# ZJU-FAST-Lab/uneven_planner

Hardware: AMD Instinct MI355X
Metric: MINCO traj-opts/sec (batch) (higher is better)
Workload: dtype f64

## Files before the change

### uneven_planner_amd/csrc/map_build.hip

```cpp
#include <hip/hip_runtime.h>
#include <hipcub/hipcub.hpp>
#include <sys/stat.h>

#include <algorithm>
#include <cmath>
#include <cstdint>
#include <chrono>
#include <cstdio>
#include <cstring>
#include <mutex>
#include <string>
#include <thread>
#include <vector>

#include "../../include/uneven_hip.h"
#include "uph_internal.hpp"
#include "terrain_dev.hpp"
#include "rccl_dyn.hpp"

using namespace uph;

struct uph_map {
    int device = 0;
    uph_map_params mp;
// ... 565 lines not shown
    g.xy_inv = 1.0 / g.xy_res; g.yaw_inv = 1.0 / g.yaw_res;
    for (int i = 0; i < 3; i++) { g.minb[i] = -size[i] / 2.0; g.maxb[i] = size[i] / 2.0; g.origin[i] = g.minb[i]; }
    finishGrid(g);
    g.nx = (int)std::ceil(size[0] / g.xy_res); g.ny = (int)std::ceil(size[1] / g.xy_res); g.nyaw = (int)std::ceil(size[2] / g.yaw_res);
    g.gravity = mp->gravity;
    if (tx1 < 0) tx1 = g.nx;
    if (tx0 < 0 || tx1 > g.nx || tx0 >= tx1) { delete m; setError("uph_map_create_tile: bad x-range"); return UPH_ERR_INVALID; }
    g.x_off = tx0; g.nx_hold = tx1 - tx0;
    m->ncell = (size_t)g.nx_hold * g.ny * g.nyaw;
    if (m->ncell >= ((size_t)1 << 31)) { setError("uph_map_create: more than 2^31 cells held by one device (the lookups index cells with 32 bits): use tiles"); delete m; return UPH_ERR_LIMIT; }
    g.cells = nullptr; g.cells32 = nullptr;
    int r = UPH_OK;
    auto alloc = [&](void** p, size_t bytes) { if (r == UPH_OK && hipMalloc(p, bytes) != hipSuccess) { setError("uph_map_create: hipMalloc of the grid failed"); r = UPH_ERR_HIP; } };
    if (f32) {
        alloc((void**)&m->d_cells32, m->ncell * 4 * sizeof(float));
        if (r == UPH_OK && hipMemset(m->d_cells32, 0, m->ncell * 4 * sizeof(float)) != hipSuccess) r = UPH_ERR_HIP;
        g.cells32 = m->d_cells32;
    } else {
        alloc((void**)&m->d_cells, m->ncell * 4 * sizeof(double));
        alloc((void**)&m->d_c, m->ncell * sizeof(double));
        if (r == UPH_OK && hipMemset(m->d_cells, 0, m->ncell * 4 * sizeof(double)) != hipSuccess) r = UPH_ERR_HIP;
        g.cells = m->d_cells;
    }
    alloc((void**)&m->d_occ, m->ncell);
    alloc((void**)&m->d_occ2, (size_t)g.nx_hold * g.ny);
    if (r == UPH_OK) r = commitMap(m);
    if (r != UPH_OK) { uph_map_destroy(m); return r; }
    *out = m;
    return UPH_OK;
}

int uph_map_create(const uph_map_params* mp, int device, uph_map** out) { return createMap(mp, device, out, false); }
int uph_map_create_f32(const uph_map_params* mp, int device, uph_map** out) { return createMap(mp, device, out, true); }
int uph_map_create_tile(const uph_map_params* mp, int device, int32_t x0, int32_t x1, int32_t f32, uph_map** out) { return createMap(mp, device, out, f32 != 0, x0, x1); }
int uph_map_tile(const uph_map* m, int32_t* x0, int32_t* x1) {
    if (!m || !x0 || !x1) return UPH_ERR_INVALID;
    *x0 = m->g.x_off; *x1 = m->g.x_off + m->g.nx_hold;
    return UPH_OK;
}
int uph_map_storage_bytes(const uph_map* m) { return !m ? UPH_ERR_INVALID : (m->d_cells32 ? 4 : 8); }

void uph_map_destroy(uph_map* m) {
    if (!m) return;
    hipSetDevice(m->device);
    hipFree(m->d_cells); hipFree(m->d_cells32); hipFree(m->d_c); hipFree(m->d_occ); hipFree(m->d_occ2);
    for (int k = 0; k < 4; k++) hipFree(m->scratch[k]);
// ... 688 lines not shown
```

### uneven_planner_amd/csrc/solver_program.hpp

```cpp
#pragma once
#include "terrain_dev.hpp"
#include "trajectory_dev.hpp"
#include "uph_common.hpp"

namespace uph {

#ifndef UPH_GRID_FROM_MEM
#define UPH_GRID_FROM_MEM 1
#endif
#ifndef UPH_PHASE_MASK
#define UPH_PHASE_MASK 15
#endif
#ifndef UPH_SCALING_WB
#define UPH_SCALING_WB 8
#endif
#ifndef UPH_SC_XB
#define UPH_SC_XB 9
#endif
#ifndef UPH_SC_YB
#define UPH_SC_YB 14
#endif
#ifndef UPH_SC_WLO
#define UPH_SC_WLO 2
#endif
#ifndef UPH_SC_WHI
#define UPH_SC_WHI 3
#endif

template <class WG, class SR = double>
struct Solver {
    WG& wg;
    const GridDev& grid;
    const OptParams& P;
    const BatchDev& bd;
    const TrajDesc& td;
    int Nxy, Nyaw, n, S, K, mem, CH, CHP, recd;
    int CHS;
// ... 300 lines not shown
    UPH_HD void putRec(int slot, int i, int j, const R gp_[2], const R gv_[2], const R ga_[2], R gyaw, R gdyaw, const KinT<R>& k) {
        rec[0 * CHP + slot] = gp_[0]; rec[1 * CHP + slot] = gp_[1];
        rec[2 * CHP + slot] = gv_[0]; rec[3 * CHP + slot] = gv_[1];
        rec[4 * CHP + slot] = ga_[0]; rec[5 * CHP + slot] = ga_[1];
        R u1 = k.u;
        if (UPH_DIET) pinv(u1);
        const R u2 = u1 * u1, u3 = u2 * u1, u4 = u2 * u2, u5 = u4 * u1;
        rec[6 * CHP + slot] = gyaw;
        rec[7 * CHP + slot] = (u1 * gyaw + gdyaw);
        rec[8 * CHP + slot] = (u2 * gyaw + 2.0 * u1 * gdyaw);
        rec[9 * CHP + slot] = (u3 * gyaw + 3.0 * u2 * gdyaw);
        rec[10 * CHP + slot] = (u4 * gyaw + 4.0 * u3 * gdyaw);
        rec[11 * CHP + slot] = (u5 * gyaw + 5.0 * u4 * gdyaw);
        rtag[slot] = k.yaw_idx;
        if (i == 0) {
            double* w = wtab + 6 * j;
            R s1 = k.s1;
            if (UPH_DIET) pinv(s1);
            const R s2 = s1 * s1, s3 = s2 * s1, s4 = s2 * s2, s5 = s4 * s1;
            w[0] = 1.0; w[1] = s1; w[2] = s2; w[3] = s3; w[4] = s4; w[5] = s5;
        }
    }

    template <int RES, class R = double>
    UPH_HD void sampleEval(int s, int slot, double* acc) {
        constexpr bool RES_ONLY = RES == 1;
        UPH_MARK("sampleEval");
        const int i = divSmall(s, K + 1, inv_k1), j = s - i * (K + 1);
        R dl[7], sc7[7];
#if !defined(UPH_LATE_DUALS) || !UPH_LATE_DUALS
#pragma unroll
        for (int q = 0; q < 7; q++) { dl[q] = R(RES_ONLY ? 0.0 : dual[q * S + s]); sc7[q] = R(scl[q * S + s]); }
#endif
        KinT<R> k;
        kin<false, R>(i, j, k);
        UPH_MARK("sampleEval.penalties");
#if defined(UPH_LATE_DUALS) && UPH_LATE_DUALS
        {
            int s_ = s;
            asm volatile("" : "+v"(s_));
#pragma unroll
            for (int q = 0; q < 7; q++) { dl[q] = R(RES_ONLY ? 0.0 : dual[q * S + s_]); sc7[q] = R(scl[q * S + s_]); }
        }
#endif
        const R icvx = k.tv[0], icvy = k.tv[2], cos_xi = k.tv[4], icxi = k.tv[5], sigma = k.tv[6];
        const R vx = k.vx, wz = k.wz, ax = k.ax, ay = k.ay, curv = k.curv_snorm;
        const R nh0 = k.syaw, nh1 = -k.cyaw;
#if defined(__HIP_DEVICE_COMPILE__) && UPH_GRID_FROM_MEM
        typedef const __attribute__((address_space(4))) unsigned long long* pw_t;
        pw_t PT = (pw_t)(const void*)bd.params_mem;
        asm volatile("" : "+s"(PT));
        constexpr int PWORD = (int)(sizeof(OptParams) / 8);
        unsigned long long pw[PWORD];
#pragma unroll
        for (int q = 0; q < PWORD; q++) pw[q] = PT[q];
        OptParams Pm;
        __builtin_memcpy(&Pm, pw, sizeof(OptParams));
#else
        const OptParams& Pm = P;
#endif
        const R h = (k.vel[0] * nh0 + k.vel[1] * nh1) * sc7[0];
        const R g1 = (vx * vx - Pm.max_vel2) * sc7[1];
        const R g2 = (ax * ax - Pm.max_acc_lon2) * sc7[2];
        const R g3 = (ay * ay - Pm.max_acc_lat2) * sc7[3];
        const R sc4 = Pm.use_scaling ? sc7[4] : R(cur_scale);
// ... 362 lines not shown
        double sm[3] = {0.0, 0.0, 0.0};
        for (int s0 = 0; s0 < S; s0 += CHS) {
            const int cnt = S - s0 < CHS ? S - s0 : CHS;
            double part[3];
            wg.template sum<3>(cnt, part, [&](int t, double* acc) { sampleObjective(s0 + t, t, acc); });
            sm[0] += part[0]; sm[1] += part[1]; sm[2] += part[2];
            scatterChunk(s0, cnt);
        }
        double chx, chy;
        adjoint(chx, chy);
        const double gTau_fx = (P.rho_T + (js[1] + sm[1] + chx) / Nxy + (js[2] + sm[2] + chy) / Nyaw) * dTau;
        const double mq = wg.maxv((Nxy - 1) * 2 + (Nyaw - 1), [&](int t) {
            return t < (Nxy - 1) * 2 ? fabs(gamxy[3 * 2 + t]) : fabs(gamyaw[3 + (t - (Nxy - 1) * 2)]);
        });
        scale_fx = wg.bcast(1.0 / dmax(1.0, dmax(mq, fabs(gTau_fx))));
        wg.pfor(2, [&](int u) { fillTimes(u); });
        wg.pfor(S, [&](int s) { scalingSample(s, dTau); });
    }

    UPH_HD void scalingSample(int s, double dTau) {
        const int i = divSmall(s, K + 1, inv_k1), j = s - i * (K + 1);
        Kin k;
        kin(i, j, k);
#if !defined(UPH_SCALING_GROUPS) || UPH_SCALING_GROUPS == 2
        scalingGroup<0, 4>(s, i, j, k, dTau);
        scalingGroup<4, 3>(s, i, j, k, dTau);
#elif UPH_SCALING_GROUPS == 3
        scalingGroup<0, 3>(s, i, j, k, dTau);
        scalingGroup<3, 2>(s, i, j, k, dTau);
        scalingGroup<5, 2>(s, i, j, k, dTau);
#else
        scalingGroup<0, 7>(s, i, j, k, dTau);
#endif
    }
    template <int Q0, int NQS>
    UPH_HD void scalingGroup(int s, int i, int j, const Kin& k, double dTau) {
        const int nbx = Nxy + 5, nby = Nyaw + 5;
        const double Tx = Txy, Ty = Tyaw, itx = 1.0 / Txy, ity = 1.0 / Tyaw;
        const double gravity = grid.gravity;
        const double alpha = 1.0 / K * j;
        const double icvx = k.tv[0], icvy = k.tv[2], icxi = k.tv[5];
        const int m = k.yaw_idx;
        double dpL[NQS][2], dvL[NQS][2], daL[NQS][2], dpR[NQS][2], dvR[NQS][2], daR[NQS][2];
        double ypL[NQS], yvL[NQS], yaL[NQS], ypR[NQS], yvR[NQS], yaR[NQS];
        double sumx[NQS], sumy[NQS], mx[NQS];
#pragma unroll
        for (int qi = 0; qi < NQS; qi++) {
// ... 312 lines not shown
        wg.pfor(S, [&](int s) {
            dual[s] += r * res[s];
            for (int q = 1; q < 7; q++) dual[q * S + s] = dmax(dual[q * S + s] + r * res[q * S + s], 0.0);
        });
        rho = wg.bcast(dmin((1 + P.gamma) * rho, P.beta));
    }
    UPH_HD bool judgeConvergence() {
        const double r = rho;
        const double rh = wg.maxv(S, [&](int s) { return fabs(res[s]); });
        const double rg = wg.maxv(6 * S, [&](int t) { return fabs(dmax(res[S + t], -dual[S + t] / r)); });
        return dmax(rh, rg) < P.epsilon_con;
    }

    UPH_HD void storeTrajectory(TrajState& st) {
        double* oc = bd.cxy + td.off_cxy;
        double* oy = bd.cyaw + td.off_cyaw;
        wg.pfor(12 * Nxy + 6 * Nyaw, [&](int t) { if (t < 12 * Nxy) oc[t] = cxy[t]; else oy[t - 12 * Nxy] = cyaw[t - 12 * Nxy]; });
        wg.pfor(1, [&](int) {
            st.T_xy = Txy; st.T_yaw = Tyaw; st.jerk_cost = last_jerk; st.scale_fx = scale_fx; st.rho = rho;
            st.evals = evals; st.hist_reads = hist_reads;
#ifdef UPH_TL_PROF
            for (int q = 0; q < 6; q++) cyc[8 + q] = wg.tl[q];
#endif
            for (int q = 0; q < 16; q++) st.cyc[q] = cyc[q];
        });
#ifdef UPH_BAR_PROF
        wg.sync();
        wg.dumpBar(&st.cyc[8]);
#endif
    }

    UPH_HD void prepare(TrajState& st) {
        const double* gx0 = bd.x0 + td.off_x;
        double* gx = bd.x + td.off_x;
        rho = wg.bcast(st.rho);
        scale_fx = 1.0;
        wg.pfor(S > n ? S : n, [&](int t) {
            if (t < n) { x[t] = gx0[t]; gx[t] = gx0[t]; }
            if (t < S) for (int q = 0; q < 7; q++) { dual[q * S + t] = 0.0; res[q * S + t] = 0.0; scl[q * S + t] = 1.0; }
        });
        const long long tstart = wg.clock();
        if (P.use_scaling) initScaling(x);
        cyc[5] += wg.clock() - tstart;
        wg.pfor(1, [&](int) { st.scale_fx = scale_fx; st.cyc[5] = cyc[5]; });
    }

    UPH_HD void optimize(TrajState& st, int cap = 0) {
// ... 211 lines not shown
```

### uneven_planner_amd/csrc/terrain_dev.hpp

```cpp
#pragma once
#include "uph_common.hpp"


namespace uph {

template <class R>
struct CornersT {
    R dx, dy, dyaw;
    uint32_t a[2][2];
    int w0, w1;
    bool inmap;
};
typedef CornersT<double> Corners;

template <class R>
UPH_HD bool isInMap(const GridDev& g, R x, R y, R yaw) {
    if (x < g.lo[0] || y < g.lo[1] || yaw < g.lo[2]) return false;
    if (x > g.hi[0] || y > g.hi[1] || yaw > g.hi[2]) return false;
    return true;
}

UPH_HD int clampIdx(int v, int hi) { return v < 0 ? 0 : (v > hi ? hi : v); }

template <class R>
// ... 39 lines not shown
    typedef const __attribute__((address_space(1))) double* wordp;
#else
    struct dbl2_t { double x, y; };
    struct flt4_t { float x, y, z, w; };
    typedef const dbl2_t* cellp;
    typedef const flt4_t* cellp32;
    typedef const double* wordp;
#endif
    if (F32) {
        const flt4_t v = ((cellp32)g.cells32)[idx];
        f[3] = toReal<R>(v.x); f[0] = toReal<R>(v.y); f[1] = toReal<R>(v.z); f[2] = toReal<R>(v.w);
    } else if (WITH_Z) {
        const cellp p = (cellp)(g.cells + 4 * (size_t)idx);
        const dbl2_t lo = p[0], hi = p[1];
        f[3] = lo.x; f[0] = lo.y; f[1] = hi.x; f[2] = hi.y;
    } else {
        const double* p = g.cells + 4 * (size_t)idx;
        const double sg = ((wordp)p)[1];
        const dbl2_t hi = ((cellp)p)[1];
        f[3] = R(0.0); f[0] = sg; f[1] = hi.x; f[2] = hi.y;
    }
}

template <bool GRAD, bool WITH_Z, class R, class CELLS>
UPH_HD void interpCellsWith(const GridDev& g, R dx, R dy, R dw, CELLS cells, R val[4], R grd[3][3]) {
    constexpr int NF = WITH_Z ? 4 : 3;
    R v0[NF], v1[NF], gy0[3], gy1[3], gx[3];
#pragma unroll
    for (int w = 0; w < 2; w++) {
        R f[2][2][4];
        cells(w, f);
#pragma unroll
        for (int k = 0; k < NF; k++) {
            const R vy0 = f[0][0][k] * (1 - dx) + f[1][0][k] * dx;
            const R vy1 = f[0][1][k] * (1 - dx) + f[1][1][k] * dx;
            const R vv = vy0 * (1 - dy) + vy1 * dy;
            if (w == 0) v0[k] = vv; else v1[k] = vv;
            if (GRAD && k < 3) {
                const R gxa = f[1][0][k] - f[0][0][k], gxb = f[1][1][k] - f[0][1][k];
                if (w == 0) { gy0[k] = vy1 - vy0; gx[k] = (1 - dw) * (1 - dy) * gxa; gx[k] += (1 - dw) * dy * gxb; }
                else { gy1[k] = vy1 - vy0; gx[k] += dw * (1 - dy) * gxa; gx[k] += dw * dy * gxb; }
            }
        }
    }
#pragma unroll
    for (int k = 0; k < NF; k++) {
        val[k] = v0[k] * (1 - dw) + v1[k] * dw;
        if (GRAD && k < 3) {
            grd[k][2] = (v1[k] - v0[k]) * g.yaw_inv;
            grd[k][1] = (gy0[k] * (1 - dw) + gy1[k] * dw) * g.xy_inv;
            grd[k][0] = gx[k] * g.xy_inv;
        }
    }
}
template <bool F32, bool GRAD, bool WITH_Z, class R>
UPH_HD void interpCells(const GridDev& g, const CornersT<R>& c, R val[4], R grd[3][3]) {
    interpCellsWith<GRAD, WITH_Z, R>(g, c.dx, c.dy, c.dyaw, [&](int w, R f[2][2][4]) {
        const int wi = w == 0 ? c.w0 : c.w1;
#pragma unroll
        for (int a = 0; a < 2; a++)
#pragma unroll
            for (int b = 0; b < 2; b++) loadCell<F32, R, WITH_Z>(g, c.a[a][b] + (uint32_t)wi, f[a][b]);
    }, val, grd);
}

template <class R>
UPH_HD void terrainBase(const GridDev& g, R x, R y, R yaw, R& sg, R& zx, R& zy, R gs[3], R gzx[3], R gzy[3]) {
    CornersT<R> c;
    locate<R>(g, x, y, yaw, c);
    sg = R(0.0); zx = R(0.0); zy = R(0.0);
#pragma unroll
    for (int k = 0; k < 3; k++) { gs[k] = R(0.0); gzx[k] = R(0.0); gzy[k] = R(0.0); }
    if (!c.inmap) return;
    R val[4], grd[3][3];
    if (g.cells32) interpCells<true, true, false, R>(g, c, val, grd);
    else interpCells<false, true, false, R>(g, c, val, grd);
    sg = val[0]; zx = val[1]; zy = val[2];
#pragma unroll
    for (int k = 0; k < 3; k++) { gs[k] = grd[0][k]; gzx[k] = grd[1][k]; gzy[k] = grd[2][k]; }
}

UPH_HD void terrainValues(const GridDev& g, const Corners& c, double val[4]) {
    val[0] = val[1] = val[2] = val[3] = 0.0;
    if (!c.inmap) return;
    double grd[3][3];
    if (g.cells32) interpCells<true, false, true, double>(g, c, val, grd);
    else interpCells<false, false, true, double>(g, c, val, grd);
}

UPH_HD void terrainAllWithGrad(const GridDev& g, double x, double y, double yaw, double cyaw, double syaw,
                               double values[7], double grads[7][3]) {
    double sg, zx, zy, gs[3], gzx[3], gzy[3];
    terrainBase(g, x, y, yaw, sg, zx, zy, gs, gzx, gzy);
    double cc = sqrt(1.0 - zx * zx - zy * zy);
    double gc[3];
#pragma unroll
    for (int k = 0; k < 3; k++) gc[k] = -(gzx[k] * zx + gzy[k] * zy) / cc;
    double inv_c = 1.0 / cc;
// ... 68 lines not shown
```

### uneven_planner_amd/csrc/unevenhip.hip

```cpp
#include <hip/hip_runtime.h>

#include <type_traits>

#include <algorithm>
#include <cmath>
#include <cstdio>
#include <cstdlib>
#include <cstring>
#include <map>
#include <numeric>
#include <string>
#include <thread>
#include <vector>

#include "../../include/uneven_hip.h"
#include "minco_op_host.hpp"
#include "resample_walk.hpp"
#include "solver_program.hpp"
#include "uph_internal.hpp"

using namespace uph;

#ifndef UPH_THOMAS_KPL
#define UPH_THOMAS_KPL 4
#endif
#ifndef UPH_WPS128
#define UPH_WPS128 2
#endif
#ifndef UPH_TWOLOOP_PF
#define UPH_TWOLOOP_PF 5
#endif

template <int CTRL>
__device__ __forceinline__ double dppMov(double v) {
    const int lo = __builtin_amdgcn_mov_dpp(__double2loint(v), CTRL, 0xf, 0xf, false);
    const int hi = __builtin_amdgcn_mov_dpp(__double2hiint(v), CTRL, 0xf, 0xf, false);
    return __hiloint2double(hi, lo);
}
__device__ __forceinline__ double readLane(double v, int l) {
    return __hiloint2double(__builtin_amdgcn_readlane(__double2hiint(v), l), __builtin_amdgcn_readlane(__double2loint(v), l));
}
__device__ __forceinline__ int uni(int v) { return __builtin_amdgcn_readfirstlane(v); }
__device__ __forceinline__ double uni(double v) {
    return __hiloint2double(__builtin_amdgcn_readfirstlane(__double2hiint(v)), __builtin_amdgcn_readfirstlane(__double2loint(v)));
}
typedef const __attribute__((address_space(1))) double* gcptr;
__device__ __forceinline__ gcptr uniG(const double* p) {
    const unsigned long long a = (unsigned long long)p;
    const unsigned lo = __builtin_amdgcn_readfirstlane((unsigned)a), hi = __builtin_amdgcn_readfirstlane((unsigned)(a >> 32));
    return (gcptr)(((unsigned long long)hi << 32) | lo);
// ... 462 lines not shown
            else if (nq == 7) twoLoopT<7, 2>(d, g, dg_out, al_lds, n, hist, m, end, bound, scale);
            else twoLoopT<8, 2>(d, g, dg_out, al_lds, n, hist, m, end, bound, scale);
            __builtin_amdgcn_s_setprio(0);
        }
        bar(1);
    }
    template <class F>
    __device__ __forceinline__ double maxv(int n, F f) {
        double a = 0.0;
        for (int i = ftid(); i < n; i += NT) { const double v = f(i); a = v > a ? v : a; }
        a = waveMax(a);
        double* r = red + par * (NW * MAXM);
        par ^= 1;
        if (lane == 0) r[wave * MAXM] = a;
        bar(0);
        double t = r[0];
#pragma unroll
        for (int w = 1; w < NW; w++) t = r[w * MAXM] > t ? r[w * MAXM] : t;
        return uni(t);
    }
};

template <int NT, int WPS, int MODE, bool F32S = false>
__global__ __launch_bounds__(NT, WPS) void uph_solver_kernel(GridDev grid, OptParams P, BatchDev bd, int repeat) {
    extern __shared__ double lds[];
    const int w = blockIdx.x;
    if (w >= bd.B) return;
    const int b = bd.order ? bd.order[w] : w;
    DevWG<NT> wg(lds);
    typedef typename std::conditional<F32S, f32r, double>::type SR;
    Solver<DevWG<NT>, SR> sol(wg, grid, P, bd, b, lds + DevWG<NT>::SCRATCH);
    TrajState& st = bd.state[b];
    if (MODE == 0) sol.evalOnly(st, repeat);
    else if (MODE == 1) sol.prepare(st);
    else if (MODE == 2) sol.optimize(st, repeat);
    else if (MODE == 7) sol.resumeHook(st, repeat >> 1, repeat & 1);
    else if (MODE == 8) { if (repeat & 1) sol.template penaltyOnly<true>(st, repeat >> 1); else sol.template penaltyOnly<false>(st, repeat >> 1); }
    else if (MODE == 3) sol.report(st);
    else if (MODE == 5) sol.microbench(st, repeat);
    else sol.scalingOnly(st);
}

__global__ void uph_fill_kernel(double* __restrict__ p, size_t n, double v) {
    for (size_t i = (size_t)blockIdx.x * blockDim.x + threadIdx.x; i < n; i += (size_t)gridDim.x * blockDim.x) p[i] = v;
}

__global__ void uph_terrain_kernel(GridDev grid, const double* __restrict__ pos, int n, double* __restrict__ values, double* __restrict__ grads) {
    const int i = blockIdx.x * blockDim.x + threadIdx.x;
    if (i >= n) return;
    const double yaw = pos[3 * i + 2];
    double v[7], g[7][3];
    terrainAllWithGrad(grid, pos[3 * i], pos[3 * i + 1], yaw, cos(yaw), sin(yaw), v, g);
    for (int k = 0; k < 7; k++) {
        values[7 * i + k] = v[k];
        for (int q = 0; q < 3; q++) grads[21 * i + 3 * k + q] = g[k][q];
    }
}

struct RolloutTraj {
    int64_t row0;
    int cnt, rows;
    double total;
    double shift[2];
// ... 219 lines not shown
    for (int k = 0; k < r.nxy; k++) {
        const double* w = states + (size_t)(r.row_xy + k) * TRAJ_STATE_COLS;
        for (int d = 0; d < 2; d++) {
            oxy[2 * k + d] = w[d];
            h.lo[d] = w[d] < h.lo[d] ? w[d] : h.lo[d];
            h.hi[d] = h.hi[d] < w[d] ? w[d] : h.hi[d];
        }
    }
    double* oyw = st_yaw + (size_t)r.q * PLAN_SY;
    double prev = h.yaw_init;
    for (int k = 0; k <= r.nyw; k++) {
        const double cur = k < r.nyw ? states[(size_t)(r.row_yaw + k) * TRAJ_STATE_COLS + 9] : h.yaw_end;
        if (k < r.nyw) oyw[k] = cur;
        const double dy = fabs(cur - prev);
        h.turn += dy; h.kink = h.kink < dy ? dy : h.kink; prev = cur;
    }
    heads[r.q] = h;
}

#ifdef UPH_ONE_KERNEL
#ifndef UPH_OK_F32
#define UPH_OK_F32 false
#endif
template __global__ void uph_solver_kernel<UPH_OK_NT, UPH_OK_WPS, UPH_OK_MODE, UPH_OK_F32>(GridDev, OptParams, BatchDev, int);
#else
namespace uph {
thread_local std::string g_last_error;
void setError(const std::string& s) { g_last_error = s; }
}

struct DevBuf {
    void* p = nullptr;
    size_t cap = 0;
    int ensure(size_t bytes) {
        if (bytes <= cap) return 0;
        if (p) hipFree(p);
        p = nullptr; cap = 0;
        size_t want = bytes + bytes / 4 + 256;
        if (hipMalloc(&p, want) != hipSuccess) { setError("hipMalloc failed"); return -1; }
        cap = want;
        return 0;
    }
    void release() { if (p) hipFree(p); p = nullptr; cap = 0; }
    template <class T> T* as() { return (T*)p; }
};

struct HostBuf {
// ... 40 lines not shown
    size_t lds_big = 0;
    int n_main = 0;
    std::vector<int> rejected;
    int n_rejected = 0;
    bool all_rejected = false;
    std::vector<TrajFrame> frames;
    std::vector<GridDev> grid_host_framed;
    GridDev frames_grid;
    GridDev framed_from;
    bool framed_valid = false;
    std::vector<int> origin;
    bool sample_f32 = false;
    int xcd_group = 0;
    hipStream_t stream2 = nullptr;
    hipEvent_t evp0 = nullptr, evp1 = nullptr;
    bool pending = false;
    hipEvent_t ev2 = nullptr;
    std::vector<size_t> fp_bytes;
    int lanes = 64;
    int lanes_forced = 0;
    int wps = 1;
    int wps_forced = 0;
    DevBuf d_thomas, d_rsd, d_rs, d_gridmem, d_parammem;
    GridDev grid_host;
    DevBuf d_desc, d_state, d_x, d_x0, d_gout, d_dual, d_res, d_scl, d_cxy, d_cyaw, d_hist, d_report, d_order, d_trace;
    DevBuf d_pen_gxy, d_pen_gyaw, d_pen_out;
    DevBuf d_roll_tt, d_roll_traj, d_roll_stage;
    bool traj_resident = false;
    DevBuf d_plan_head, d_plan_xy, d_plan_yaw, d_plan_goal, d_plan_rec;
    bool planned = false;
    std::vector<ProblemHead> plan_probs;
    std::vector<double> end_pose;
    std::vector<double> end_bnd;
    DevBuf d_sw_q, d_sw_out;
    DevBuf d_refine_rec;
    int trace_cap = 0;
    int trace_cap_up = 0;
    std::vector<TrajState> state_host;
    HostBuf h_x, h_cxy, h_cyaw, h_dual, h_res, h_scl;
    double last_ms = 0.0, last_prepare_ms = 0.0;
    int64_t last_evals = 0, last_sample_evals = 0, last_iters = 0, last_hist_bytes = 0;
};

#define HIPCHK(call)                                                                               \
    do {                                                                                           \
        hipError_t _e = (call);                                                                    \
// ... 64 lines not shown
        }
        if (!c->framed_valid || std::memcmp(&c->framed_from, &grid, sizeof(GridDev)) != 0) {
            if (c->d_gridmem.ensure(sizeof(GridDev) * c->frames.size())) return UPH_ERR_HIP;
            c->grid_host_framed.assign(c->frames.size(), grid);
            for (size_t b = 0; b < c->frames.size(); b++) applyFrame(c->grid_host_framed[b], c->frames[b]);
            HIPCHK(hipMemcpyAsync(c->d_gridmem.p, c->grid_host_framed.data(), sizeof(GridDev) * c->frames.size(), hipMemcpyHostToDevice, c->stream));
            c->framed_from = grid;
            c->framed_valid = true;
        }
    }
    return UPH_OK;
}

static int launchSolver(uph_ctx* c, int mode, int repeat, bool async = false, hipEvent_t evb = nullptr, hipEvent_t eve = nullptr) {
    if (!async && c->pending) { setError("an asynchronous solve is in flight on this context: call uph_batch_wait first"); return UPH_ERR_INVALID; }
    if (!evb) { evb = c->ev0; eve = c->ev1; }
    HIPCHK(hipSetDevice(uphMapDevice(c->map)));
    GridDev grid;
    const int rg = syncGridMem(c, grid);
    if (rg != UPH_OK) return rg;
    if (c->d_parammem.ensure(sizeof(OptParams))) return UPH_ERR_HIP;
    HIPCHK(hipMemcpyAsync(c->d_parammem.p, &c->P, sizeof(OptParams), hipMemcpyHostToDevice, c->stream));
    BatchDev bd = makeBatchDev(c);
#define UPH_LAUNCH(NTL, WPS, MODE)                                                                                                     \
    do {                                                                                                                             \
        const size_t ldsmax = 160 * 1024;    \
        HIPCHK(hipFuncSetAttribute((const void*)uph_solver_kernel<NTL, WPS, MODE>, hipFuncAttributeMaxDynamicSharedMemorySize, (int)ldsmax)); \
        HIPCHK(hipEventRecord(evb, c->stream));                                                                                   \
        BatchDev bm = bd;                                                                                                            \
        bm.B = c->n_main;                                                                                                            \
        if (c->n_main < c->B) {            \
            BatchDev bb = bd;              \
            bb.B = c->B - c->n_main;                                                                                                 \
            bb.order = bd.order + c->n_main;                                                                                         \
            HIPCHK(hipStreamWaitEvent(c->stream2, evb, 0));                                                                       \
            hipLaunchKernelGGL((uph_solver_kernel<NTL, WPS, MODE>), dim3(bb.B), dim3(NTL), c->lds_big, c->stream2, grid, c->P, bb, repeat); \
            HIPCHK(hipEventRecord(c->ev2, c->stream2));                                                                              \
        }                                                                                                                            \
        hipLaunchKernelGGL((uph_solver_kernel<NTL, WPS, MODE>), dim3(c->n_main), dim3(NTL), c->lds_bytes, c->stream, grid, c->P, bm, repeat); \
        if (c->n_main < c->B) HIPCHK(hipStreamWaitEvent(c->stream, c->ev2, 0));                                                      \
    } while (0)
#define UPH_LAUNCH_MODE(NTL, WPS)                                                                                                      \
    do {                                                                                                                             \
        if (mode == 0) UPH_LAUNCH(NTL, WPS, 0);                                                                                      \
        else if (mode == 1) UPH_LAUNCH(NTL, WPS, 1);                                                                                 \
        else if (mode == 2) UPH_LAUNCH(NTL, WPS, 2);                                                                                 \
        else if (mode == 3) UPH_LAUNCH(NTL, WPS, 3);                                                                                 \
        else if (mode == 5) UPH_LAUNCH(NTL, WPS, 5);                                                                                 \
        else UPH_LAUNCH(NTL, WPS, 4);                                                                                                \
    } while (0)
#define UPH_LAUNCH32(NTL, WPS, MODE)                                                                                                   \
    do {                                                                                                                             \
        const size_t ldsmax = 160 * 1024;    \
        HIPCHK(hipFuncSetAttribute((const void*)uph_solver_kernel<NTL, WPS, MODE, true>, hipFuncAttributeMaxDynamicSharedMemorySize, (int)ldsmax)); \
        HIPCHK(hipEventRecord(evb, c->stream));                                                                                   \
        BatchDev bm = bd;                                                                                                            \
        bm.B = c->n_main;                                                                                                            \
        if (c->n_main < c->B) {                                                                                                      \
            BatchDev bb = bd;                                                                                                        \
            bb.B = c->B - c->n_main;                                                                                                 \
            bb.order = bd.order + c->n_main;                                                                                         \
            HIPCHK(hipStreamWaitEvent(c->stream2, evb, 0));                                                                       \
            hipLaunchKernelGGL((uph_solver_kernel<NTL, WPS, MODE, true>), dim3(bb.B), dim3(NTL), c->lds_big, c->stream2, grid, c->P, bb, repeat); \
            HIPCHK(hipEventRecord(c->ev2, c->stream2));                                                                              \
        }                                                                                                                            \
        hipLaunchKernelGGL((uph_solver_kernel<NTL, WPS, MODE, true>), dim3(c->n_main), dim3(NTL), c->lds_bytes, c->stream, grid, c->P, bm, repeat); \
        if (c->n_main < c->B) HIPCHK(hipStreamWaitEvent(c->stream, c->ev2, 0));                                                      \
    } while (0)
    if (c->sample_f32 && (mode == 0 || mode == 2) && (c->lanes == 128 || c->lanes == 256 || c->lanes == 512)) {
        if (c->lanes == 128) { if (mode == 0) UPH_LAUNCH32(128, 2, 0); else UPH_LAUNCH32(128, 2, 2); }
        else if (c->lanes == 512) { if (mode == 0) UPH_LAUNCH32(512, 1, 0); else UPH_LAUNCH32(512, 1, 2); }
        else if (mode == 0) UPH_LAUNCH32(256, 1, 0);
        else if (c->wps == 2 && c->lds_bytes <= 80 * 1024) UPH_LAUNCH32(256, 2, 2);
        else UPH_LAUNCH32(256, 1, 2);
    }
    else if (mode == 7) {
        if (c->lanes == 128) UPH_LAUNCH(128, 2, 7);
        else if (c->lanes == 256) UPH_LAUNCH(256, 1, 7);
        else { setError("the L-BFGS resume hook is built for 128 and 256 lanes"); return UPH_ERR_INVALID; }
    }
    else if (mode == 8) {
        if (c->lanes == 128) UPH_LAUNCH(128, 2, 8);
        else if (c->lanes == 256) UPH_LAUNCH(256, 1, 8);
        else if (c->lanes == 512) UPH_LAUNCH(512, 1, 8);
        else UPH_LAUNCH(64, 1, 8);
    }
    else if (c->lanes == 64 && c->wps_forced == 2) UPH_LAUNCH_MODE(64, 2);
    else if (c->lanes == 64) UPH_LAUNCH_MODE(64, 1);
    else if (c->lanes == 128 && mode == 1) UPH_LAUNCH(128, 1, 1);
// ... 61 lines not shown
        buildThomasTable(tab);
        if (c->d_thomas.ensure(tab.size() * sizeof(double))) { delete c; return UPH_ERR_HIP; }
        if (hipMemcpy(c->d_thomas.p, tab.data(), tab.size() * sizeof(double), hipMemcpyHostToDevice) != hipSuccess) { setError("hipMemcpy(thomas table) failed"); c->d_thomas.release(); delete c; return UPH_ERR_HIP; }
    }
    HIPCHK(hipStreamCreateWithFlags(&c->stream, hipStreamNonBlocking));
    {
        int prio_lo = 0, prio_hi = 0;
        hipDeviceGetStreamPriorityRange(&prio_lo, &prio_hi);
        HIPCHK(hipStreamCreateWithPriority(&c->stream2, hipStreamNonBlocking, prio_hi));
    }
    HIPCHK(hipEventCreate(&c->ev2));
    HIPCHK(hipEventCreate(&c->evp0)); HIPCHK(hipEventCreate(&c->evp1));
    HIPCHK(hipEventCreate(&c->ev0));
    HIPCHK(hipEventCreate(&c->ev1));
    *out = c;
    return UPH_OK;
}

void uph_ctx_destroy(uph_ctx* c) {
    if (!c) return;
    hipSetDevice(c->device);
    for (void* p : c->op_allocs) hipFree(p);
    DevBuf* bufs[] = {&c->d_ops, &c->d_desc, &c->d_state, &c->d_x, &c->d_gout, &c->d_dual, &c->d_res, &c->d_scl, &c->d_cxy, &c->d_cyaw,
                      &c->d_hist, &c->d_report, &c->d_order, &c->d_trace, &c->d_x0, &c->d_thomas, &c->d_rsd, &c->d_rs, &c->d_gridmem, &c->d_parammem,
                      &c->d_pen_gxy, &c->d_pen_gyaw, &c->d_pen_out, &c->d_roll_tt, &c->d_roll_traj, &c->d_roll_stage,
                      &c->d_plan_head, &c->d_plan_xy, &c->d_plan_yaw, &c->d_plan_goal, &c->d_plan_rec, &c->d_sw_q, &c->d_sw_out, &c->d_refine_rec};
    for (DevBuf* b : bufs) b->release();
    HostBuf* hbufs[] = {&c->h_x, &c->h_cxy, &c->h_cyaw, &c->h_dual, &c->h_res, &c->h_scl};
    for (HostBuf* b : hbufs) b->release();
    if (c->ev0) hipEventDestroy(c->ev0);
    if (c->ev1) hipEventDestroy(c->ev1);
    if (c->stream) hipStreamDestroy(c->stream);
    if (c->stream2) hipStreamDestroy(c->stream2);
    if (c->ev2) hipEventDestroy(c->ev2);
    if (c->evp0) hipEventDestroy(c->evp0);
    if (c->evp1) hipEventDestroy(c->evp1);
    delete c;
}

int uph_ctx_set_lanes(uph_ctx* c, int32_t lanes) {
    if (!c || (lanes != 0 && lanes != 64 && lanes != 128 && lanes != 256 && lanes != 512)) return UPH_ERR_INVALID;
    c->lanes_forced = lanes;
    return UPH_OK;
}
int uph_ctx_set_xcd_locality(uph_ctx* c, int32_t group) { if (!c || group < 0) return UPH_ERR_INVALID; c->xcd_group = group; return UPH_OK; }
int uph_ctx_set_wps(uph_ctx* c, int32_t wps) { if (!c || wps < 0 || wps > 2) return UPH_ERR_INVALID; c->wps_forced = wps; return UPH_OK; }
int uph_ctx_set_sample_precision(uph_ctx* c, int32_t bits) {
// ... 1181 lines not shown
```

### uneven_planner_amd/csrc/uph_common.hpp

```cpp
#pragma once
#include <math.h>
#include <stdint.h>

#if defined(__HIPCC__)
#define UPH_HD __host__ __device__ __forceinline__
#define UPH_NOINLINE __host__ __device__ __attribute__((noinline))
#else
#define UPH_HD inline
#define UPH_NOINLINE __attribute__((noinline))
#endif

#if defined(__HIP_DEVICE_COMPILE__)
#define UPH_AS_GLOBAL(p) ((const __attribute__((address_space(1))) double*)(p))
#else
#define UPH_AS_GLOBAL(p) (p)
#endif

#if defined(UPH_ISA_MARKS) && defined(__HIP_DEVICE_COMPILE__)
#define UPH_MARK(name) asm volatile("; UPHMARK " name)
#else
#define UPH_MARK(name) do { } while (0)
#endif

namespace uph {

constexpr int MAX_PIECE_XY = 128;
constexpr int MAX_PIECE_YAW = 256;
constexpr int MAX_MEM = 256;
constexpr int MAX_PAST = 8;

constexpr double delta_sigl = 0.01;
constexpr double cur_scale = 10.0;
constexpr double sig_scale = 1000.0;
constexpr double scale_trick_jerk = 1000.0;

enum {
    LBFGS_CONVERGENCE = 0,
    LBFGS_STOP,
    LBFGS_CANCELED,
    LBFGSERR_UNKNOWNERROR = -1024,
    LBFGSERR_INVALID_N,
    LBFGSERR_INVALID_MEMSIZE,
    LBFGSERR_INVALID_GEPSILON,
    LBFGSERR_INVALID_TESTPERIOD,
    LBFGSERR_INVALID_DELTA,
    LBFGSERR_INVALID_MINSTEP,
    LBFGSERR_INVALID_MAXSTEP,
    LBFGSERR_INVALID_FDECCOEFF,
    LBFGSERR_INVALID_SCURVCOEFF,
    LBFGSERR_INVALID_MACHINEPREC,
    LBFGSERR_INVALID_MAXLINESEARCH,
    LBFGSERR_INVALID_FUNCVAL,
    LBFGSERR_MINIMUMSTEP,
    LBFGSERR_MAXIMUMSTEP,
    LBFGSERR_MAXIMUMLINESEARCH,
    LBFGSERR_MAXIMUMITERATION,
    LBFGSERR_WIDTHTOOSMALL,
    LBFGSERR_INVALIDPARAMETERS,
    LBFGSERR_INCREASEGRADIENT,
};

struct GridDev {
    int nx, ny, nyaw;
    int x_off, nx_hold;
    int ix_off = 0, iy_off = 0;
    double xy_res, yaw_res, xy_inv, yaw_inv;
    double origin[3], minb[3], maxb[3];
    double lo[3], hi[3];
    double half_xy, half_yaw;
    double gravity;
    const double* cells;
    const float* cells32;
};

struct OptParams {
    double rho_T, rho_ter, max_vel, max_acc_lon, max_acc_lat, max_kap, min_cxi, max_sig;
    int use_scaling;
    double beta, gamma, epsilon_con, max_iter;
    double g_epsilon, min_step, delta;
    int inner_max_iter, mem_size, past, int_K;
    int max_linesearch;
    double max_step, f_dec_coeff, s_curv_coeff, cautious_factor, machine_prec;
    double max_vel2, max_acc_lon2, max_acc_lat2, max_kap2;
};

inline void finishGrid(GridDev& g) {
    for (int i = 0; i < 3; i++) { g.lo[i] = g.minb[i] + 1e-4; g.hi[i] = g.maxb[i] - 1e-4; }
    g.half_xy = 0.5 * g.xy_res; g.half_yaw = 0.5 * g.yaw_res;
}
inline void finishParams(OptParams& P) {
    P.max_vel2 = P.max_vel * P.max_vel; P.max_acc_lon2 = P.max_acc_lon * P.max_acc_lon;
    P.max_acc_lat2 = P.max_acc_lat * P.max_acc_lat; P.max_kap2 = P.max_kap * P.max_kap;
}

struct MincoOp {
    int N;
    const double* Wt;
    const double* Wr;
};

constexpr double FRAME_EXTENT = 32.0;
struct TrajFrame {
    double fo[2];
    double lo[2], hi[2];
    double shift[2];
    int ioff[2];
};
inline void applyFrame(GridDev& g, const TrajFrame& f) {
// ... 215 lines not shown
```

Measured before the change: 50260.

## Use buffer-resource loads for grid cells and duals, retune scaling groups, add tickets

Grid-cell and dual/scale loads now go through AMD buffer resources with 32-bit offsets, used whenever the held grid fits in 4 GB, in place of 64-bit global address arithmetic. The scaling-sample split defaults to three groups and the scaling work-block constant drops from 8 to 4. An optional atomic ticket scheme for dynamic workgroup ordering is added but off by default, along with XCD trace instrumentation. The buffer loads are meant to cut address VALU work and register pressure. A risk is that buffer-resource bounds and flags differ from plain global loads, and the numeric sizes (computed as signed int) could overflow near the 4 GB edge.

```diff
diff --git a/uneven_planner_amd/csrc/map_build.hip b/uneven_planner_amd/csrc/map_build.hip
--- a/uneven_planner_amd/csrc/map_build.hip
+++ b/uneven_planner_amd/csrc/map_build.hip
@@ -611,6 +611,7 @@
         if (r == UPH_OK && hipMemset(m->d_cells, 0, m->ncell * 4 * sizeof(double)) != hipSuccess) r = UPH_ERR_HIP;
         g.cells = m->d_cells;
     }
+    g.off32 = gridOffsetForm(g);
     alloc((void**)&m->d_occ, m->ncell);
     alloc((void**)&m->d_occ2, (size_t)g.nx_hold * g.ny);
     if (r == UPH_OK) r = commitMap(m);
diff --git a/uneven_planner_amd/csrc/solver_program.hpp b/uneven_planner_amd/csrc/solver_program.hpp
--- a/uneven_planner_amd/csrc/solver_program.hpp
+++ b/uneven_planner_amd/csrc/solver_program.hpp
@@ -12,7 +12,13 @@
 #define UPH_PHASE_MASK 15
 #endif
 #ifndef UPH_SCALING_WB
-#define UPH_SCALING_WB 8
+#define UPH_SCALING_WB 4
+#endif
+#ifndef UPH_SCALING_GROUPS
+#define UPH_SCALING_GROUPS 3
+#endif
+#ifndef UPH_OFF32_DUALS
+#define UPH_OFF32_DUALS 1
 #endif
 #ifndef UPH_SC_XB
 #define UPH_SC_XB 9
@@ -359,6 +365,23 @@
         }
     }
 
+    template <bool RES_ONLY, class R>
+    UPH_HD void loadDuals(int s, R dl[7], R sc7[7]) const {
+#if defined(__HIP_DEVICE_COMPILE__) && UPH_OFF32_DUALS
+        const uint32_t plane = (uint32_t)S * 8u, so = (uint32_t)s * 8u;
+        const __amdgpu_buffer_rsrc_t rd = __builtin_amdgcn_make_buffer_rsrc((void*)dual, 0, (int)(7u * plane), 0x00020000);
+        const __amdgpu_buffer_rsrc_t rs = __builtin_amdgcn_make_buffer_rsrc((void*)scl, 0, (int)(7u * plane), 0x00020000);
+#pragma unroll
+        for (int q = 0; q < 7; q++) {
+            dl[q] = R(RES_ONLY ? 0.0 : __builtin_bit_cast(double, __builtin_amdgcn_raw_buffer_load_b64(rd, (int)so, (int)((uint32_t)q * plane), 0)));
+            sc7[q] = R(__builtin_bit_cast(double, __builtin_amdgcn_raw_buffer_load_b64(rs, (int)so, (int)((uint32_t)q * plane), 0)));
+        }
+#else
+#pragma unroll
+        for (int q = 0; q < 7; q++) { dl[q] = R(RES_ONLY ? 0.0 : dual[q * S + s]); sc7[q] = R(scl[q * S + s]); }
+#endif
+    }
+
     template <int RES, class R = double>
     UPH_HD void sampleEval(int s, int slot, double* acc) {
         constexpr bool RES_ONLY = RES == 1;
@@ -366,8 +389,7 @@
         const int i = divSmall(s, K + 1, inv_k1), j = s - i * (K + 1);
         R dl[7], sc7[7];
 #if !defined(UPH_LATE_DUALS) || !UPH_LATE_DUALS
-#pragma unroll
-        for (int q = 0; q < 7; q++) { dl[q] = R(RES_ONLY ? 0.0 : dual[q * S + s]); sc7[q] = R(scl[q * S + s]); }
+        loadDuals<RES_ONLY, R>(s, dl, sc7);
 #endif
         KinT<R> k;
         kin<false, R>(i, j, k);
@@ -376,8 +398,7 @@
         {
             int s_ = s;
             asm volatile("" : "+v"(s_));
-#pragma unroll
-            for (int q = 0; q < 7; q++) { dl[q] = R(RES_ONLY ? 0.0 : dual[q * S + s_]); sc7[q] = R(scl[q * S + s_]); }
+            loadDuals<RES_ONLY, R>(s_, dl, sc7);
         }
 #endif
         const R icvx = k.tv[0], icvy = k.tv[2], cos_xi = k.tv[4], icxi = k.tv[5], sigma = k.tv[6];
@@ -786,7 +807,7 @@
         const int i = divSmall(s, K + 1, inv_k1), j = s - i * (K + 1);
         Kin k;
         kin(i, j, k);
-#if !defined(UPH_SCALING_GROUPS) || UPH_SCALING_GROUPS == 2
+#if UPH_SCALING_GROUPS == 2
         scalingGroup<0, 4>(s, i, j, k, dTau);
         scalingGroup<4, 3>(s, i, j, k, dTau);
 #elif UPH_SCALING_GROUPS == 3
@@ -1145,7 +1166,7 @@
 #ifdef UPH_TL_PROF
             for (int q = 0; q < 6; q++) cyc[8 + q] = wg.tl[q];
 #endif
-            for (int q = 0; q < 16; q++) st.cyc[q] = cyc[q];
+            for (int q = 0; q < (UPH_XCD_TRACE ? 13 : 16); q++) st.cyc[q] = cyc[q];
         });
 #ifdef UPH_BAR_PROF
         wg.sync();
diff --git a/uneven_planner_amd/csrc/terrain_dev.hpp b/uneven_planner_amd/csrc/terrain_dev.hpp
--- a/uneven_planner_amd/csrc/terrain_dev.hpp
+++ b/uneven_planner_amd/csrc/terrain_dev.hpp
@@ -85,6 +85,54 @@
     }
 }
 
+struct CellBuf {
+#if defined(__HIP_DEVICE_COMPILE__)
+    __amdgpu_buffer_rsrc_t r;
+#else
+    const char* base;
+#endif
+};
+template <bool F32>
+UPH_HD CellBuf cellBuf(const GridDev& g) {
+    CellBuf cb;
+#if defined(__HIP_DEVICE_COMPILE__)
+    const uint32_t bytes = (uint32_t)g.nx_hold * (uint32_t)g.ny * (uint32_t)g.nyaw * (F32 ? 16u : 32u);
+    cb.r = __builtin_amdgcn_make_buffer_rsrc(F32 ? (void*)g.cells32 : (void*)g.cells, 0, (int)bytes, 0x00020000);
+#else
+    cb.base = F32 ? (const char*)g.cells32 : (const char*)g.cells;
+#endif
+    return cb;
+}
+template <bool F32, class R, bool WITH_Z = true>
+UPH_HD void loadCellOff(const CellBuf& cb, uint32_t idx, R f[4]) {
+    const uint32_t off = idx << (F32 ? 4 : 5);
+#if defined(__HIP_DEVICE_COMPILE__)
+    typedef double dbl2_t __attribute__((ext_vector_type(2)));
+    typedef float flt4_t __attribute__((ext_vector_type(4)));
+    if (F32) {
+        const flt4_t v = __builtin_bit_cast(flt4_t, __builtin_amdgcn_raw_buffer_load_b128(cb.r, (int)off, 0, 0));
+        f[3] = toReal<R>(v.x); f[0] = toReal<R>(v.y); f[1] = toReal<R>(v.z); f[2] = toReal<R>(v.w);
+    } else if (WITH_Z) {
+        const dbl2_t lo = __builtin_bit_cast(dbl2_t, __builtin_amdgcn_raw_buffer_load_b128(cb.r, (int)off, 0, 0));
+        const dbl2_t hi = __builtin_bit_cast(dbl2_t, __builtin_amdgcn_raw_buffer_load_b128(cb.r, (int)(off + 16u), 0, 0));
+        f[3] = lo.x; f[0] = lo.y; f[1] = hi.x; f[2] = hi.y;
+    } else {
+        const double sg = __builtin_bit_cast(double, __builtin_amdgcn_raw_buffer_load_b64(cb.r, (int)(off + 8u), 0, 0));
+        const dbl2_t hi = __builtin_bit_cast(dbl2_t, __builtin_amdgcn_raw_buffer_load_b128(cb.r, (int)(off + 16u), 0, 0));
+        f[3] = R(0.0); f[0] = sg; f[1] = hi.x; f[2] = hi.y;
+    }
+#else
+    const char* p = cb.base + off;
+    if (F32) {
+        const float* v = (const float*)p;
+        f[3] = toReal<R>(v[0]); f[0] = toReal<R>(v[1]); f[1] = toReal<R>(v[2]); f[2] = toReal<R>(v[3]);
+    } else {
+        const double* v = (const double*)p;
+        f[3] = WITH_Z ? R(v[0]) : R(0.0); f[0] = v[1]; f[1] = v[2]; f[2] = v[3];
+    }
+#endif
+}
+
 template <bool GRAD, bool WITH_Z, class R, class CELLS>
 UPH_HD void interpCellsWith(const GridDev& g, R dx, R dy, R dw, CELLS cells, R val[4], R grd[3][3]) {
     constexpr int NF = WITH_Z ? 4 : 3;
@@ -116,14 +164,19 @@
         }
     }
 }
-template <bool F32, bool GRAD, bool WITH_Z, class R>
+template <bool F32, bool GRAD, bool WITH_Z, class R, bool OFF32 = false>
 UPH_HD void interpCells(const GridDev& g, const CornersT<R>& c, R val[4], R grd[3][3]) {
+    CellBuf cb;
+    if (OFF32) cb = cellBuf<F32>(g);
     interpCellsWith<GRAD, WITH_Z, R>(g, c.dx, c.dy, c.dyaw, [&](int w, R f[2][2][4]) {
         const int wi = w == 0 ? c.w0 : c.w1;
 #pragma unroll
         for (int a = 0; a < 2; a++)
 #pragma unroll
-            for (int b = 0; b < 2; b++) loadCell<F32, R, WITH_Z>(g, c.a[a][b] + (uint32_t)wi, f[a][b]);
+            for (int b = 0; b < 2; b++) {
+                if (OFF32) loadCellOff<F32, R, WITH_Z>(cb, c.a[a][b] + (uint32_t)wi, f[a][b]);
+                else loadCell<F32, R, WITH_Z>(g, c.a[a][b] + (uint32_t)wi, f[a][b]);
+            }
     }, val, grd);
 }
 
@@ -136,7 +189,9 @@
     for (int k = 0; k < 3; k++) { gs[k] = R(0.0); gzx[k] = R(0.0); gzy[k] = R(0.0); }
     if (!c.inmap) return;
     R val[4], grd[3][3];
-    if (g.cells32) interpCells<true, true, false, R>(g, c, val, grd);
+    if (g.off32 == 1) interpCells<false, true, false, R, true>(g, c, val, grd);
+    else if (g.off32 == 2) interpCells<true, true, false, R, true>(g, c, val, grd);
+    else if (g.cells32) interpCells<true, true, false, R>(g, c, val, grd);
     else interpCells<false, true, false, R>(g, c, val, grd);
     sg = val[0]; zx = val[1]; zy = val[2];
 #pragma unroll
diff --git a/uneven_planner_amd/csrc/unevenhip.hip b/uneven_planner_amd/csrc/unevenhip.hip
--- a/uneven_planner_amd/csrc/unevenhip.hip
+++ b/uneven_planner_amd/csrc/unevenhip.hip
@@ -26,6 +26,9 @@
 #endif
 #ifndef UPH_WPS128
 #define UPH_WPS128 2
+#endif
+#ifndef UPH_TICKETS_DEFAULT
+#define UPH_TICKETS_DEFAULT 0
 #endif
 #ifndef UPH_TWOLOOP_PF
 #define UPH_TWOLOOP_PF 5
@@ -534,11 +537,21 @@
 };
 
 template <int NT, int WPS, int MODE, bool F32S = false>
-__global__ __launch_bounds__(NT, WPS) void uph_solver_kernel(GridDev grid, OptParams P, BatchDev bd, int repeat) {
+__global__ __launch_bounds__(NT, WPS) void uph_solver_kernel(GridDev grid, OptParams P, BatchDev bd, int repeat, int* __restrict__ ticket) {
     extern __shared__ double lds[];
-    const int w = blockIdx.x;
+    int w = blockIdx.x;
     if (w >= bd.B) return;
+    if (MODE == 2 && ticket != nullptr) {
+        int* slot = (int*)lds;
+        if (threadIdx.x == 0) *slot = atomicAdd(ticket, 1);
+        __syncthreads();
+        w = uni(*slot);
+        __syncthreads();
+    }
     const int b = bd.order ? bd.order[w] : w;
+#if UPH_XCD_TRACE
+    const long long t_enter = (long long)wall_clock64();
+#endif
     DevWG<NT> wg(lds);
     typedef typename std::conditional<F32S, f32r, double>::type SR;
     Solver<DevWG<NT>, SR> sol(wg, grid, P, bd, b, lds + DevWG<NT>::SCRATCH);
@@ -551,6 +564,13 @@
     else if (MODE == 3) sol.report(st);
     else if (MODE == 5) sol.microbench(st, repeat);
     else sol.scalingOnly(st);
+#if UPH_XCD_TRACE
+    if (MODE == 2 && threadIdx.x == 0) {
+        st.cyc[13] = (long long)__builtin_amdgcn_s_getreg((3 << 11) | 20);
+        st.cyc[14] = t_enter;
+        st.cyc[15] = (long long)wall_clock64();
+    }
+#endif
 }
 
 __global__ void uph_fill_kernel(double* __restrict__ p, size_t n, double v) {
@@ -816,7 +836,7 @@
 #ifndef UPH_OK_F32
 #define UPH_OK_F32 false
 #endif
-template __global__ void uph_solver_kernel<UPH_OK_NT, UPH_OK_WPS, UPH_OK_MODE, UPH_OK_F32>(GridDev, OptParams, BatchDev, int);
+template __global__ void uph_solver_kernel<UPH_OK_NT, UPH_OK_WPS, UPH_OK_MODE, UPH_OK_F32>(GridDev, OptParams, BatchDev, int, int*);
 #else
 namespace uph {
 thread_local std::string g_last_error;
@@ -903,6 +923,7 @@
     int wps = 1;
     int wps_forced = 0;
     DevBuf d_thomas, d_rsd, d_rs, d_gridmem, d_parammem;
+    DevBuf d_ticket;
     GridDev grid_host;
     DevBuf d_desc, d_state, d_x, d_x0, d_gout, d_dual, d_res, d_scl, d_cxy, d_cyaw, d_hist, d_report, d_order, d_trace;
     DevBuf d_pen_gxy, d_pen_gyaw, d_pen_out;
@@ -1013,6 +1034,13 @@
     if (c->d_parammem.ensure(sizeof(OptParams))) return UPH_ERR_HIP;
     HIPCHK(hipMemcpyAsync(c->d_parammem.p, &c->P, sizeof(OptParams), hipMemcpyHostToDevice, c->stream));
     BatchDev bd = makeBatchDev(c);
+    const char* tk = std::getenv("UNEVENHIP_TICKETS");
+    const bool use_tickets = tk && *tk ? std::atoi(tk) != 0 : UPH_TICKETS_DEFAULT != 0;
+    int* ticket = nullptr;
+    if (mode == 2 && use_tickets) {
+        if (c->d_ticket.ensure(2 * sizeof(int))) return UPH_ERR_HIP;
+        ticket = c->d_ticket.as<int>();
+    }
 #define UPH_LAUNCH(NTL, WPS, MODE)                                                                                                     \
     do {                                                                                                                             \
         const size_t ldsmax = 160 * 1024;    \
@@ -1025,10 +1053,12 @@
             bb.B = c->B - c->n_main;                                                                                                 \
             bb.order = bd.order + c->n_main;                                                                                         \
             HIPCHK(hipStreamWaitEvent(c->stream2, evb, 0));                                                                       \
-            hipLaunchKernelGGL((uph_solver_kernel<NTL, WPS, MODE>), dim3(bb.B), dim3(NTL), c->lds_big, c->stream2, grid, c->P, bb, repeat); \
+            if (ticket) HIPCHK(hipMemsetAsync(ticket + 1, 0, sizeof(int), c->stream2));                                              \
+            hipLaunchKernelGGL((uph_solver_kernel<NTL, WPS, MODE>), dim3(bb.B), dim3(NTL), c->lds_big, c->stream2, grid, c->P, bb, repeat, ticket ? ticket + 1 : nullptr); \
             HIPCHK(hipEventRecord(c->ev2, c->stream2));                                                                              \
         }                                                                                                                            \
-        hipLaunchKernelGGL((uph_solver_kernel<NTL, WPS, MODE>), dim3(c->n_main), dim3(NTL), c->lds_bytes, c->stream, grid, c->P, bm, repeat); \
+        if (ticket) HIPCHK(hipMemsetAsync(ticket, 0, sizeof(int), c->stream));                                                       \
+        hipLaunchKernelGGL((uph_solver_kernel<NTL, WPS, MODE>), dim3(c->n_main), dim3(NTL), c->lds_bytes, c->stream, grid, c->P, bm, repeat, ticket); \
         if (c->n_main < c->B) HIPCHK(hipStreamWaitEvent(c->stream, c->ev2, 0));                                                      \
     } while (0)
 #define UPH_LAUNCH_MODE(NTL, WPS)                                                                                                      \
@@ -1052,10 +1082,12 @@
             bb.B = c->B - c->n_main;                                                                                                 \
             bb.order = bd.order + c->n_main;                                                                                         \
             HIPCHK(hipStreamWaitEvent(c->stream2, evb, 0));                                                                       \
-            hipLaunchKernelGGL((uph_solver_kernel<NTL, WPS, MODE, true>), dim3(bb.B), dim3(NTL), c->lds_big, c->stream2, grid, c->P, bb, repeat); \
+            if (ticket) HIPCHK(hipMemsetAsync(ticket + 1, 0, sizeof(int), c->stream2));                                              \
+            hipLaunchKernelGGL((uph_solver_kernel<NTL, WPS, MODE, true>), dim3(bb.B), dim3(NTL), c->lds_big, c->stream2, grid, c->P, bb, repeat, ticket ? ticket + 1 : nullptr); \
             HIPCHK(hipEventRecord(c->ev2, c->stream2));                                                                              \
         }                                                                                                                            \
-        hipLaunchKernelGGL((uph_solver_kernel<NTL, WPS, MODE, true>), dim3(c->n_main), dim3(NTL), c->lds_bytes, c->stream, grid, c->P, bm, repeat); \
+        if (ticket) HIPCHK(hipMemsetAsync(ticket, 0, sizeof(int), c->stream));                                                       \
+        hipLaunchKernelGGL((uph_solver_kernel<NTL, WPS, MODE, true>), dim3(c->n_main), dim3(NTL), c->lds_bytes, c->stream, grid, c->P, bm, repeat, ticket); \
         if (c->n_main < c->B) HIPCHK(hipStreamWaitEvent(c->stream, c->ev2, 0));                                                      \
     } while (0)
     if (c->sample_f32 && (mode == 0 || mode == 2) && (c->lanes == 128 || c->lanes == 256 || c->lanes == 512)) {
@@ -1163,7 +1195,7 @@
     hipSetDevice(c->device);
     for (void* p : c->op_allocs) hipFree(p);
     DevBuf* bufs[] = {&c->d_ops, &c->d_desc, &c->d_state, &c->d_x, &c->d_gout, &c->d_dual, &c->d_res, &c->d_scl, &c->d_cxy, &c->d_cyaw,
-                      &c->d_hist, &c->d_report, &c->d_order, &c->d_trace, &c->d_x0, &c->d_thomas, &c->d_rsd, &c->d_rs, &c->d_gridmem, &c->d_parammem,
+                      &c->d_hist, &c->d_report, &c->d_order, &c->d_trace, &c->d_x0, &c->d_thomas, &c->d_rsd, &c->d_rs, &c->d_gridmem, &c->d_parammem, &c->d_ticket,
                       &c->d_pen_gxy, &c->d_pen_gyaw, &c->d_pen_out, &c->d_roll_tt, &c->d_roll_traj, &c->d_roll_stage,
                       &c->d_plan_head, &c->d_plan_xy, &c->d_plan_yaw, &c->d_plan_goal, &c->d_plan_rec, &c->d_sw_q, &c->d_sw_out, &c->d_refine_rec};
     for (DevBuf* b : bufs) b->release();
diff --git a/uneven_planner_amd/csrc/uph_common.hpp b/uneven_planner_amd/csrc/uph_common.hpp
--- a/uneven_planner_amd/csrc/uph_common.hpp
+++ b/uneven_planner_amd/csrc/uph_common.hpp
@@ -20,6 +20,10 @@
 #define UPH_MARK(name) asm volatile("; UPHMARK " name)
 #else
 #define UPH_MARK(name) do { } while (0)
+#endif
+
+#ifndef UPH_XCD_TRACE
+#define UPH_XCD_TRACE 0
 #endif
 
 namespace uph {
@@ -64,6 +68,7 @@
     int nx, ny, nyaw;
     int x_off, nx_hold;
     int ix_off = 0, iy_off = 0;
+    int off32 = 0;
     double xy_res, yaw_res, xy_inv, yaw_inv;
     double origin[3], minb[3], maxb[3];
     double lo[3], hi[3];
@@ -84,6 +89,10 @@
     double max_vel2, max_acc_lon2, max_acc_lat2, max_kap2;
 };
 
+inline int gridOffsetForm(const GridDev& g) {
+    const unsigned long long bytes = (unsigned long long)g.nx_hold * g.ny * g.nyaw * (g.cells32 ? 16u : 32u);
+    return bytes < (1ull << 32) ? (g.cells32 ? 2 : 1) : 0;
+}
 inline void finishGrid(GridDev& g) {
     for (int i = 0; i < 3; i++) { g.lo[i] = g.minb[i] + 1e-4; g.hi[i] = g.maxb[i] - 1e-4; }
     g.half_xy = 0.5 * g.xy_res; g.half_yaw = 0.5 * g.yaw_res;
```

Result: slower. 49730 (-1.1%).
